# CCIG-Champalimaud/adell-mri

Hardware: AMD Instinct MI355X
Metric: volumes/sec 3D U-Net 128^3 2-ch seg (train step: fwd+loss+bwd+SGD) (higher is better)
Workload: dtype f32 (f16x3 split MFMA, fp32 accumulate); 1 GPU; BASELINE configs[1]: u-net-3d-resnet.yaml UNetPL, 2x128^3, batch 2/GPU, dice+focal, SGD-Nesterov; per_gpu_batch=2, parallelism=dp1, yaml=configs/u-net-3d-resnet.yaml, built_by=parse_config_unet -> get_segmentation_network('unet'), gradient_exchange=none (1 rank)

## Files before the change

adell_mri_amd/_lib.py:

```python
import ctypes
import os

_HERE = os.path.dirname(os.path.abspath(__file__))
LIB_PATH = os.environ.get("ADELL_HIP_LIBRARY") or os.path.join(_HERE, "libadellhip.so")

_lib = None

OK = 0
E_BADARG, E_UNSUPPORTED, E_HIP, E_NOMEM = -1, -2, -3, -4

ACT_IDS = {
    "identity": 0, "swish": 1, "silu": 1, "relu": 2, "leaky_relu": 3, "prelu": 4,
    "gelu": 5, "sigmoid": 6, "tanh": 7, "elu": 8,
}


class AdellHipError(RuntimeError):
    pass


class ConvDesc(ctypes.Structure):
    _fields_ = [(n, ctypes.c_int32) for n in (
        "N", "D", "H", "W", "C0", "C1", "Cout", "KD", "KH", "KW", "SD", "SH", "SW",
        "PD", "PH", "PW", "Do", "Ho", "Wo")]
# ... 93 lines not shown
    "adell_dice_focal_workspace": (_l, [_i, _l]),
    "adell_dice_focal_fwd": (_i, [_vp, _vp, _i, _l, _f, _f, _f, _f, _f, _vp, _vp, _vp, _vp, ctypes.c_size_t, _vp]),
    "adell_dice_focal_bwd": (_i, [_vp, _vp, _i, _l, _f, _f, _f, _f, _f, _vp, _f, _f, _vp, _vp]),
    "adell_dice_focal_bwd_dev": (_i, [_vp, _vp, _i, _l, _f, _f, _f, _f, _f, _vp, _vp, _vp, _vp, _vp]),
    "adell_class_sums_workspace": (_l, [_i, _l, _i]),
    "adell_class_sums_fwd": (_i, [_vp, _vp, _i, _l, _i, _vp, _vp, ctypes.c_size_t, _vp]),
    "adell_class_sums_bwd": (_i, [_vp, _vp, _i, _l, _i, _vp, _vp]),
    "adell_sgd_step": (_i, [_vp, _vp, _vp, _l, _f, _f, _f, _i, _i, _f, _vp]),
    "adell_adamw_step": (_i, [_vp, _vp, _vp, _vp, _l, _f, _f, _f, _f, _f, _l, _f, _vp]),
    "adell_adam_step": (_i, [_vp, _vp, _vp, _vp, _l, _f, _f, _f, _f, _f, _l, _f, _vp]),
    "adell_ema_update": (_i, [_vp, _vp, _l, _f, _vp]),
    "adell_layernorm_fwd": (_i, [_vp, _vp, _vp, _vp, _vp, _vp, _l, _i, _f, _vp]),
    "adell_layernorm_bwd_workspace": (_l, [_l, _i]),
    "adell_layernorm_bwd": (_i, [_vp] * 8 + [_l, _i, _vp, ctypes.c_size_t, _vp]),
    "adell_add_bcast": (_i, [_vp, _vp, _vp, _l, _l, _vp]),
    "adell_sum_bcast": (_i, [_vp, _vp, _l, _l, _vp]),
    "adell_attention_fwd": (_i, [_vp, _vp, _vp, _vp, _i, _i, _i, _i, _i, _f, _f, ctypes.c_ulonglong,
                                 ctypes.c_uint, _vp, _vp, _vp]),
    "adell_attention_bwd": (_i, [_vp, _vp, _vp, _vp, _i, _vp, _vp, _vp, _i, _i, _i, _i, _f, _f,
                                 ctypes.c_ulonglong, ctypes.c_uint, _vp, _vp, _vp, _vp]),
    "adell_attention_strided_ok": (_i, [_i, _i, _i]),
    "adell_attention_fwd_strided": (_i, [_vp, _vp, _vp, _vp, _i, _i, _i, _i, _i, _i, _vp, _f, _f,
                                         ctypes.c_ulonglong, ctypes.c_uint, _vp, _vp, _vp]),
    "adell_attention_bwd_strided": (_i, [_vp, _vp, _vp, _vp, _i, _vp, _vp, _vp, _i, _i, _i, _i, _i,
                                         _vp, _f, _f, ctypes.c_ulonglong, ctypes.c_uint, _vp, _vp,
                                         _vp, _vp]),
    "adell_copy_channels": (_i, [_vp, _vp, _l, _i, _i, _i, _i, _vp]),
    "adell_interp_nearest_fwd": (_i, [_vp, _vp] + [_i] * 8 + [_vp]),
    "adell_interp_nearest_bwd": (_i, [_vp, _vp] + [_i] * 8 + [_vp]),
    "adell_interp_linear_fwd": (_i, [_vp, _vp] + [_i] * 8 + [_f] * 3 + [_i, _vp]),
    "adell_interp_linear_bwd": (_i, [_vp, _vp] + [_i] * 8 + [_f] * 3 + [_i, _vp]),
    "adell_fold_x_taps": (_i, [_vp, _vp] + [_i] * 8 + [_vp]),
    "adell_scale_bc": (_i, [_vp, _vp, _vp, _i, _l, _i, _vp]),
    "adell_scale_bc_dscale_workspace_floats": (_l, [_i, _l, _i]),
    "adell_scale_bc_dscale": (_i, [_vp, _vp, _vp, _i, _l, _i, _vp, _vp]),
    "adell_cse_apply": (_i, [_vp, _vp, _vp, _vp, _vp, _vp, _i, _l, _i, _vp]),
    "adell_cse_apply_bwd_workspace_floats": (_l, [_i, _l, _i]),
    "adell_cse_apply_bwd": (_i, [_vp, _vp, _vp, _vp, _vp, _vp, _vp, _vp, _i, _l, _i, _vp, _vp]),
    "adell_bcast_nc": (_i, [_vp, _vp, _i, _l, _i, _f, _vp]),
    "adell_maxpool3d_fwd": (_i, [ctypes.POINTER(ConvDesc), _vp, _vp, _vp, _vp]),
    "adell_maxpool3d_bwd": (_i, [ctypes.POINTER(ConvDesc), _vp, _vp, _vp, _vp]),
    "adell_dwconv3d_fwd": (_i, [_i] * 8 + [_vp] * 5),
    "adell_dwconv3d_bwd_data": (_i, [_i] * 8 + [_vp] * 4),
    "adell_dwconv3d_bwd_weight_workspace_floats": (_l, [_i] * 8),
    "adell_dwconv3d_bwd_weight": (_i, [_i] * 8 + [_vp] * 6),
    "adell_vicreg_scratch_floats": (_l, [_i, _i]),
    "adell_vicreg_fwd": (_i, [_vp, _vp, _i, _i, _f, _f, _vp, _vp, _vp]),
    "adell_vicreg_bwd": (_i, [_vp, _vp, _i, _i, _f, _f, _vp, _vp, _vp, _vp, _vp]),
    "adell_convt_k2_applicable": (_i, [_i] * 6),
    "adell_convt_k2_fwd": (_i, [_i] * 6 + [_vp] * 5),
    "adell_convt_k2_bwd_data": (_i, [_i] * 6 + [_vp] * 4),
    "adell_convt_k2_wgrad_workspace": (_l, [_i] * 6),
    "adell_convt_k2_bwd_weight": (_i, [_i] * 6 + [_vp] * 5 + [ctypes.c_size_t, _vp]),
    "adell_convt_k221_applicable": (_i, [_i] * 6),
    "adell_convt_k221_fwd": (_i, [_i] * 6 + [_vp] * 5),
    "adell_convt_k221_bwd_data": (_i, [_i] * 6 + [_vp] * 4),
    "adell_convt_k221_wgrad_workspace": (_l, [_i] * 6),
    "adell_convt_k221_bwd_weight": (_i, [_i] * 6 + [_vp] * 5 + [ctypes.c_size_t, _vp]),
    "adell_conv_cinfold_applicable": (_i, [ctypes.POINTER(ConvDesc)]),
    "adell_conv_cinfold_ntiles": (_i, [ctypes.POINTER(ConvDesc)]),
    "adell_conv_cinfold_fwd": (_i, [ctypes.POINTER(ConvDesc)] + [_vp] * 5 + [_i, _vp]),
    "adell_conv_cinfold_fwd_f16x3": (_i, [ctypes.POINTER(ConvDesc)] + [_vp] * 5 + [_i, _vp]),
    "adell_conv_cinfold_wgrad_workspace": (_l, [ctypes.POINTER(ConvDesc)]),
    "adell_conv_cinfold_bwd_weight": (_i, [ctypes.POINTER(ConvDesc)] + [_vp] * 5
                                      + [ctypes.c_size_t, _vp]),
    "adell_conv_cinfold_bwd_weight_f16x3": (_i, [ctypes.POINTER(ConvDesc)] + [_vp] * 5
                                            + [ctypes.c_size_t, _vp]),
    "adell_conv_cinfold_dx_applicable": (_i, [ctypes.POINTER(ConvDesc)]),
    "adell_conv_cinfold_bwd_data": (_i, [ctypes.POINTER(ConvDesc)] + [_vp] * 4),
    "adell_conv_cinfold_bwd_data_f16x3": (_i, [ctypes.POINTER(ConvDesc)] + [_vp] * 4),
    "adell_pair_loss_scratch_floats": (_l, [_i, _i]),
    "adell_pair_loss_fwd": (_i, [_vp, _vp, _i, _i, _i, _f, _i, _vp, _vp, _vp]),
    "adell_pair_loss_bwd": (_i, [_vp, _vp, _i, _i, _i, _f, _i, _vp, _vp, _vp, _vp, _vp]),
    "adell_loco_loss_workspace": (_l, [_i, _l, _i]),
    "adell_loco_loss_fwd": (_i, [_vp, _vp, _i, _l, _i, _f, _f, _vp, _vp, ctypes.c_size_t, _vp]),
    "adell_loco_loss_bwd": (_i, [_vp, _vp, _vp, _i, _l, _i, _f, _f, _vp, _vp, _vp]),
    "adell_prelu_wgrad_workspace": (_l, [ctypes.POINTER(NormActDesc)]),
    "adell_prelu_wgrad": (_i, [ctypes.POINTER(NormActDesc)] + [_vp] * 8 + [ctypes.c_size_t, _vp]),
    "adell_convtranspose3d_fwd_f16x3": (_i, [_i] * 9 + [_vp] * 7),
    "adell_convtranspose3d_bwd_data_f16x3": (_i, [_i] * 9 + [_vp] * 6),
    "adell_convtranspose3d_f16x3_plan": (_i, [_i] * 9 + [_vp]),
    "adell_conv1_small_applicable": (_i, [ctypes.POINTER(ConvDesc)]),
    "adell_conv1_small_fwd": (_i, [ctypes.POINTER(ConvDesc)] + [_vp] * 6),
    "adell_conv1_small_bwd_data": (_i, [ctypes.POINTER(ConvDesc)] + [_vp] * 5),
    "adell_conv1_small_wgrad_workspace": (_l, [ctypes.POINTER(ConvDesc)]),
    "adell_conv1_small_bwd_weight": (_i, [ctypes.POINTER(ConvDesc)] + [_vp] * 6 + [ctypes.c_size_t, _vp]),
    "adell_conv_cin_small_applicable": (_i, [ctypes.POINTER(ConvDesc)]),
    "adell_conv_cin_small_ntiles": (_i, [ctypes.POINTER(ConvDesc)]),
    "adell_conv_cin_small_fwd": (_i, [ctypes.POINTER(ConvDesc)] + [_vp] * 5 + [_i, _vp]),
    "adell_conv_cin_small_bwd_data": (_i, [ctypes.POINTER(ConvDesc)] + [_vp] * 4),
    "adell_multi_copy": (_i, [_vp, _i, _vp, _vp]),
    "adell_grad_norm_workspace": (_l, [_i]),
    "adell_grad_norm_partials": (_i, [_vp, _l, _i, _vp, _i, _vp]),
    "adell_grad_norm_finalize": (_i, [_vp, _i, _i, _f, _f, _vp, _vp]),
    "adell_grad_scale_by": (_i, [_vp, _l, _vp, _vp]),
    "adell_multi_accumulate": (_i, [_vp, _i, _vp, _vp]),
    "adell_seg_confusion_workspace": (_l, [_l, _i]),
    "adell_seg_confusion_update": (_i, [_vp, _vp, _i, _l, _i, _l, _i, _vp, _l, _vp, _i, _vp]),
    "adell_seg_metric_compute": (_i, [_vp, _i, _i, _f, _vp, _vp]),
    "adell_cc_workspace": (_l, [_l, _i, _i, _i]),
    "adell_cc_label": (_i, [_vp, _l, _i, _i, _i, _i, _f, _vp, _vp, _vp, _l, _vp]),
    "adell_picai_tables_workspace": (_l, [_l, _i, _i, _i]),
    "adell_picai_tables_capacity": (_l, [_l, _i, _i, _i]),
    "adell_picai_tables": (_i, [_vp, _vp, _l, _i, _i, _i, _i, _f, _vp, _vp, _l, _vp, _l, _vp]),
    "adell_item_stats_workspace": (_l, [_i, _l]),
    "adell_item_stats": (_i, [_vp, _i, _l, _vp, _vp, ctypes.c_size_t, _vp]),
# ... 97 lines not shown
```

adell_mri_amd/csrc/convt_k2.hip:

```cpp
#include "common.h"

struct ConvTK2Args {
  const float* x;
  const float* w;
  const float* bias;
  const float* dy;
  float* y;
  float* dx;
  float* ws;
  float* wsdb;
  int N, D, H, W, Cin, Cout;
  int FX;
  long V;
  int ntiles;
};

__device__ __forceinline__ size_t adell_ctk2_fine(const ConvTK2Args& a, long v64, int fz, int fy) {
  const unsigned v = (unsigned)v64, W = (unsigned)a.W, H = (unsigned)a.H, D = (unsigned)a.D;
  const unsigned t1 = v / W, x = v - t1 * W;
  const unsigned t2 = t1 / H, y = t1 - t2 * H;
  const unsigned n = t2 / D, z = t2 - n * D;
  return (((size_t)n * 2 * D + 2 * z + fz) * 2 * H + 2 * y + fy) * (size_t)(a.FX * W) + (size_t)a.FX * x;
}

// ... 197 lines not shown
  float4 dbacc = make_float4(0.f, 0.f, 0.f, 0.f);
  auto fetch = [&](int t) {
    const long v0 = (long)t * 32;
    const int valid = (a.V - v0) < 32 ? (int)(a.V - v0) : 32;
    const size_t yrow = li < valid ? adell_ctk2_fine(a, v0 + li, fz, fy) * a.Cout : 0;
    adell_ctk2_fetch<32>(rx, valid, lane, a.x + (size_t)v0 * a.Cin + ci0, (size_t)li * a.Cin);
    adell_ctk2_fetch<32>(ry0, valid, lane, a.dy, yrow, co0);
    if constexpr (FX == 2) adell_ctk2_fetch<32>(ry1, valid, lane, a.dy, yrow, a.Cout + co0);
  };
  if ((int)blockIdx.x < a.ntiles) fetch(blockIdx.x);
  for (int t = blockIdx.x; t < a.ntiles; t += gridDim.x) {
    adell_ctk2_put<32>(tx, LDX, lane, rx);
    adell_ctk2_put<32>(tyl, LDY, lane, ry0);
    if constexpr (FX == 2) adell_ctk2_put<32>(tyl + 32, LDY, lane, ry1);
    if (do_db) {
#pragma unroll
      for (int u = 0; u < CtK2Regs<32>::PER; ++u) {
        dbacc.x += ry0.f[u].x; dbacc.y += ry0.f[u].y; dbacc.z += ry0.f[u].z; dbacc.w += ry0.f[u].w;
        if constexpr (FX == 2) {
          dbacc.x += ry1.f[u].x; dbacc.y += ry1.f[u].y; dbacc.z += ry1.f[u].z; dbacc.w += ry1.f[u].w;
        }
      }
    }
    __builtin_amdgcn_s_waitcnt(0xc07f);
    if (t + (int)gridDim.x < a.ntiles) fetch(t + gridDim.x);
#pragma unroll
    for (int s = 0; s < 16; ++s) {
      const int v = 2 * s + lh;
      const float av = tx[v * LDX + li];
#pragma unroll
      for (int fx = 0; fx < FX; ++fx)
        acc[fx] = __builtin_amdgcn_mfma_f32_32x32x2f32(av, tyl[v * LDY + fx * 32 + li], acc[fx],
                                                        0, 0, 0);
    }
  }
  float* out = a.ws + (((size_t)blockIdx.x * gridDim.y + blockIdx.y) * (4 * FX)) * 1024;
#pragma unroll
  for (int fx = 0; fx < FX; ++fx)
#pragma unroll
    for (int r = 0; r < 16; ++r) {
      const int row = (r & 3) + 8 * (r >> 2) + 4 * lh;
      out[(size_t)((fz * 2 + fy) * FX + fx) * 1024 + row * 32 + li] = acc[fx][r];
    }
  if (do_db) {
#pragma unroll
    for (int o = 8; o < 64; o <<= 1) {
      dbacc.x += __shfl_xor(dbacc.x, o, 64);
      dbacc.y += __shfl_xor(dbacc.y, o, 64);
      dbacc.z += __shfl_xor(dbacc.z, o, 64);
      dbacc.w += __shfl_xor(dbacc.w, o, 64);
    }
    if (lane < 8) {
      float* o = a.wsdb + ((size_t)blockIdx.x * 4 + wave) * a.Cout + co0 + 4 * lane;
      o[0] = dbacc.x; o[1] = dbacc.y; o[2] = dbacc.z; o[3] = dbacc.w;
    }
  }
}

__global__ __launch_bounds__(256) void adell_convt_k2_dw16_kernel(ConvTK2Args a) {
  constexpr int LDX = 33, LDY = 33;
  __shared__ float sx[4][32 * LDX];
  __shared__ float sy[4][32 * LDY];
  const int lane = threadIdx.x & 63, wave = threadIdx.x >> 6, li = lane & 31, lh = lane >> 5;
  const int fz = wave >> 1, fy = wave & 1;
  const int ci0 = blockIdx.y * 32;
  f32x16 acc;
#pragma unroll
  for (int r = 0; r < 16; ++r) acc[r] = 0.f;
  float* tx = sx[wave];
  float* tyl = sy[wave];
  CtK2Regs<32> rx, ry;
  const bool do_db = a.wsdb != nullptr && ci0 == 0;
  float4 dbacc = make_float4(0.f, 0.f, 0.f, 0.f);
  auto fetch = [&](int t) {
    const long v0 = (long)t * 32;
    const int valid = (a.V - v0) < 32 ? (int)(a.V - v0) : 32;
    const size_t yrow = li < valid ? adell_ctk2_fine(a, v0 + li, fz, fy) * 16 : 0;
    adell_ctk2_fetch<32>(rx, valid, lane, a.x + (size_t)v0 * a.Cin + ci0, (size_t)li * a.Cin);
    adell_ctk2_fetch<32>(ry, valid, lane, a.dy, yrow);
  };
  if ((int)blockIdx.x < a.ntiles) fetch(blockIdx.x);
  for (int t = blockIdx.x; t < a.ntiles; t += gridDim.x) {
    adell_ctk2_put<32>(tx, LDX, lane, rx);
    adell_ctk2_put<32>(tyl, LDY, lane, ry);
    if (do_db) {
#pragma unroll
      for (int u = 0; u < CtK2Regs<32>::PER; ++u) {
        dbacc.x += ry.f[u].x; dbacc.y += ry.f[u].y; dbacc.z += ry.f[u].z; dbacc.w += ry.f[u].w;
      }
    }
    __builtin_amdgcn_s_waitcnt(0xc07f);
    if (t + (int)gridDim.x < a.ntiles) fetch(t + gridDim.x);
#pragma unroll
    for (int s = 0; s < 16; ++s) {
      const int v = 2 * s + lh;
      acc = __builtin_amdgcn_mfma_f32_32x32x2f32(tx[v * LDX + li], tyl[v * LDY + li], acc, 0, 0, 0);
    }
  }
  float* out = a.ws + (((size_t)blockIdx.x * gridDim.y + blockIdx.y) * 4 + (fz * 2 + fy)) * 1024;
#pragma unroll
  for (int r = 0; r < 16; ++r) {
    const int row = (r & 3) + 8 * (r >> 2) + 4 * lh;
    out[row * 32 + li] = acc[r];
  }
  if (do_db) {
#pragma unroll
// ... 174 lines not shown
  return adell_convt_k2_wgrad_ws_impl(N, D, H, W, Cin, Cout, 1);
}

static int adell_convt_k2_bwd_weight_impl(int N, int D, int H, int W, int Cin, int Cout, int FX,
                                          const float* x, const float* dy, float* dw, float* db,
                                          void* workspace, size_t workspace_bytes, void* stream) {
  ADELL_REQUIRE(x && dy && dw && workspace && adell_convt_k2_ok(N, D, H, W, Cin, Cout, FX),
                "convt_k2_bwd_weight: factor-2 transposed conv with 32 / 64 channels expected");
  ADELL_REQUIRE((((uintptr_t)x | (uintptr_t)dy) & 15) == 0,
                "convt_k2_bwd_weight: x and dy must be 16-byte aligned");
  ADELL_REQUIRE((long)workspace_bytes >= adell_convt_k2_wgrad_ws_impl(N, D, H, W, Cin, Cout, FX),
                "convt_k2_bwd_weight: workspace too small");
  ConvTK2Args a = {};
  adell_ctk2_fill(&a, N, D, H, W, Cin, Cout, FX);
  a.x = x; a.dy = dy; a.ws = (float*)workspace;
  const int blocks = adell_ctk2_blocks(a, 2);
  hipStream_t st = (hipStream_t)stream;
  if (Cout == 16) {
    a.wsdb = db ? a.ws + (size_t)blocks * (Cin / 32) * 4 * 1024 : nullptr;
    hipLaunchKernelGGL(adell_convt_k2_dw16_kernel, dim3((unsigned)blocks, (unsigned)(Cin / 32)), dim3(256),
                       0, st, a);
    const long outs16 = (long)Cin * 16 * 8 + (db ? 16 : 0);
    hipLaunchKernelGGL(adell_convt_k2_dw16_reduce_kernel, dim3((unsigned)((outs16 + 3) / 4)), dim3(256),
                       0, st, (const float*)workspace, blocks, Cin, dw, (const float*)a.wsdb, db);
    ADELL_CHECK_HIP(hipGetLastError());
    return ADELL_OK;
  }
  const int F = 4 * FX;
  a.wsdb = db ? a.ws + (size_t)blocks * (Cin / 32) * (Cout / 32) * F * 1024 : nullptr;
  dim3 grid((unsigned)blocks, (unsigned)((Cin / 32) * (Cout / 32)));
  if (FX == 2)
    hipLaunchKernelGGL(adell_convt_k2_dw_kernel<2>, grid, dim3(256), 0, st, a);
  else
    hipLaunchKernelGGL(adell_convt_k2_dw_kernel<1>, grid, dim3(256), 0, st, a);
  const long outs = (long)Cin * Cout * F + (db ? Cout : 0);
  hipLaunchKernelGGL(adell_convt_k2_dw_reduce_kernel, dim3((unsigned)((outs + 3) / 4)), dim3(256), 0,
                     st, (const float*)workspace, blocks, Cin, Cout, dw, (const float*)a.wsdb, db, F);
  ADELL_CHECK_HIP(hipGetLastError());
  return ADELL_OK;
}

extern "C" int adell_convt_k2_bwd_weight(int N, int D, int H, int W, int Cin, int Cout,
                                         const float* x, const float* dy, float* dw, float* db,
                                         void* workspace, size_t workspace_bytes, void* stream) {
  return adell_convt_k2_bwd_weight_impl(N, D, H, W, Cin, Cout, 2, x, dy, dw, db, workspace,
                                        workspace_bytes, stream);
}
extern "C" int adell_convt_k221_bwd_weight(int N, int D, int H, int W, int Cin, int Cout,
                                           const float* x, const float* dy, float* dw, float* db,
                                           void* workspace, size_t workspace_bytes, void* stream) {
  return adell_convt_k2_bwd_weight_impl(N, D, H, W, Cin, Cout, 1, x, dy, dw, db, workspace,
                                        workspace_bytes, stream);
}
```

adell_mri_amd/functional.py:

```python
import itertools
import os
import weakref

import numpy as np
import torch
import torch.distributed as dist

from . import _lib, ops

_dropout_counter = itertools.count(1)

CONV_PRECISION = os.environ.get("ADELL_CONV_PRECISION", "f16x3")
FLAGS = {"s2class_always": bool(os.environ.get("ADELL_S2CLASS_ALWAYS")),
         "no_s2class": bool(os.environ.get("ADELL_NO_S2CLASS")),
         "no_fold": bool(os.environ.get("ADELL_NO_FOLD")),
         "no_adn_fuse": bool(os.environ.get("ADELL_NO_ADN_FUSE")),
         "no_lowrank": bool(os.environ.get("ADELL_NO_LOWRANK")),
         "wgrad_stream": os.environ.get("ADELL_WGRAD_STREAM", "1") != "0",
         "no_rows": bool(os.environ.get("ADELL_NO_ROWS")),
         "no_pointwise_gemm": bool(os.environ.get("ADELL_NO_POINTWISE_GEMM")),
         "no_seq_attention": bool(os.environ.get("ADELL_NO_SEQ_ATTENTION")),
         "no_mlp_fuse": not bool(os.environ.get("ADELL_MLP_FUSE")),
         "mlp_min_elems": int(os.environ.get("ADELL_MLP_MIN_ELEMS", str(1 << 20))),
         "no_cinfold_wgrad_f16": bool(os.environ.get("ADELL_NO_CINFOLD_WGRAD_F16"))}


def set_conv_precision(mode):
    global CONV_PRECISION
    if mode not in ("f16x3", "fp32"):
        raise ValueError("conv precision must be 'f16x3' or 'fp32'")
    CONV_PRECISION = mode
    _sync_dw_precision()


def _sync_dw_precision():
    from . import _lib
    if os.path.exists(_lib.LIB_PATH) and not os.environ.get("ADELL_DW_NOMFMA"):
        _lib.lib().adell_set_tuning(b"dw_nomfma", 1 if CONV_PRECISION == "fp32" else 0)


if CONV_PRECISION == "fp32":
    _sync_dw_precision()


class _Ref:

    __slots__ = ("obj",)

    def __init__(self, obj):
        self.obj = obj


_PACK_REG = {}
_PACK_BATCH = {"epoch": -1, "sig": None, "table": None, "blocks": 0}


class _PackFence:

    __slots__ = ("stream", "event")

    def __init__(self):
        self.stream = ops._stream().value
        self.event = torch.cuda.Event()
        self.event.record()

    def order(self):
        if ops._stream().value != self.stream:
            torch.cuda.current_stream().wait_event(self.event)


def _pack_tag(w):
    return (w._version, w.data_ptr(), ops.WEIGHT_EPOCH)


def _repack_registered():
    live = []
    for key, ent in list(_PACK_REG.items()):
# ... 626 lines not shown
    adn = _adn_sites_of(x0, x1, weight, stride, padding)
    rows0 = getattr(x0, "_adell_rows", None)
    rows1 = getattr(x1, "_adell_rows", None) if x1 is not None else None
    conf = (stride, padding, want_stats, _Ref(weight), carry_in, carry_out, carry_x0, carry_cat,
            adn, rows0, rows1)
    Cin = x0.shape[1] + (0 if x1 is None else x1.shape[1])
    small1 = ops.conv1_small_ok(weight, Cin, stride, padding, residual)
    if small1:
        wp = None
        site = getattr(x0, "_adell_site", None) if getattr(x0, "_adell_single", False) else None
        if (site is not None and x1 is None and carry_in is None and carry_x0 is None
                and not grad_observed(x0)
                and not FLAGS["no_adn_fuse"] and not FLAGS["no_lowrank"]
                and torch.is_grad_enabled() and ops.norm_act_lowrank_ok(x0, weight.shape[0])):
            conf = conf[:8] + (("lowrank", site),) + conf[9:]
    elif ops.conv_cin_small_ok(weight, x0, x1, stride, padding, residual):
        wp = "cin_small"
    elif ops.conv_cinfold_ok(weight, x0, x1, stride, padding, residual):
        wp = "cinfold"
    elif (CONV_PRECISION == "f16x3" and x1 is None and weight.dim() == 5 and x0.shape[1] <= 4
          and 3 <= weight.shape[4] and weight.shape[4] * x0.shape[1] <= 16
          and stride == (1, 1, 1) and not FLAGS["no_fold"]):
        wp = ("fold", _packed_folded(weight))
    else:
        wp = _packed(weight, 0)
    y, part = _Conv3dFn.apply(x0, x1, weight, bias, residual, wp, conf)
    if want_stats and part.numel() > 0:
        y._adell_partials = part
    return y


class _ConvT3dFn(torch.autograd.Function):
    @staticmethod
    def forward(ctx, x, weight, bias, wp, wref):
        factors = tuple(weight.shape[2:])
        ctx.k2 = wp is None
        if ctx.k2:
            y = ops.convt_k2_fwd(x, weight, bias)
        else:
            y = ops.convtranspose3d_fwd(x, wp, bias, weight.shape[1], factors)
        ctx.save_for_backward(x, weight)
        ctx.has_bias = bias is not None
        ctx.bias_ref = _Ref(bias)
        ctx.wref = wref
        ctx.factors = factors
        return y

    @staticmethod
    def backward(ctx, dy):
        x, weight = ctx.saved_tensors
        need = ctx.needs_input_grad
        dy = ops.ndhwc(dy)
        dx = dw = db = None
        if need[0]:
            dx = (ops.convt_k2_bwd_data(dy, weight) if ctx.k2 else
                  ops.convtranspose3d_bwd_data(dy, _packed(ctx.wref.obj, 3), weight.shape[0],
                                               ctx.factors))
        want_db = ctx.has_bias and need[2]

        def weight_grads():
            dw = db = None
            if need[1] and ctx.k2 and want_db:
                dw, db = ops.convt_k2_bwd_weight(x, dy, want_db=True, factors=ctx.factors)
            elif need[1]:
                dw = (ops.convt_k2_bwd_weight(x, dy, factors=ctx.factors) if ctx.k2 else
                      ops.convtranspose3d_bwd_weight(x, dy, ctx.factors))
            if want_db and db is None:
                db = ops.bias_grad(dy)
            return dw, db

        if (need[1] or want_db) and _side_ok(ctx.wref.obj, ctx.bias_ref.obj):
            dw, db = side_run(weight_grads, (x, dy))
        else:
            dw, db = weight_grads()
        return dx, dw, db, None, None


def conv_transpose3d(x, weight, bias=None):
    wp = None if (x.dim() == 5 and ops.convt_k2_ok(x.shape, weight)) else _packed(weight, 2)
    _note_use(weight)
    return _ConvT3dFn.apply(x, weight, bias, wp, _Ref(weight))


conv_transpose3d_k2s2 = conv_transpose3d


class _NormDropActFn(torch.autograd.Function):
    @staticmethod
    def forward(ctx, x, mean, rstd, gamma, beta, act_w, conf):
        act, act_p, per_item, drop_p, seed, offset, site, split_exp, _group = conf
        if site is not None:
            out, mask = ops.norm_act_fwd(x, mean, rstd, act, gamma=gamma, beta=beta, act_w=act_w,
                                         act_p=act_p, stats_per_item=per_item, drop_p=drop_p,
                                         seed=seed, rng_offset=offset, want_mask=True,
                                         split_exp=split_exp)
            site.x, site.mean, site.rstd, site.mask = x, mean, rstd, mask
        else:
            out = ops.norm_act_fwd(x, mean, rstd, act, gamma=gamma, beta=beta, act_w=act_w,
                                   act_p=act_p, stats_per_item=per_item, drop_p=drop_p, seed=seed,
                                   rng_offset=offset, split_exp=split_exp)
        ctx.save_for_backward(x, mean, rstd, gamma, beta, act_w)
        ctx.conf = conf
        return out

    @staticmethod
    def backward(ctx, dout):
        x, mean, rstd, gamma, beta, act_w = ctx.saved_tensors
        act, act_p, per_item, drop_p, seed, offset, site, _split_exp, group = ctx.conf
        if site is not None:
            fused, part, poff = site.fused, site.part, site.poff
            site.fused, site.part = False, None
# ... 948 lines not shown
```

adell_mri_amd/ops.py:

```python
import collections
import ctypes
import math
import os

import torch

from . import _lib
from ._lib import ACT_IDS, AdellHipError, ConvDesc, NormActDesc, check


class KernelTimer:

    def __init__(self, only=None):
        self.records = []
        self._agg = None
        self.only = None if only is None else set(only)
        self.active = True

    def start(self):
        e = torch.cuda.Event(enable_timing=True)
        e.record()
        return e

    def stop(self, name, flops, e0, tag=None, nbytes=0.0, kernels=1):
# ... 751 lines not shown
    N, Cin, D, H, W = x.shape
    Cout = weight.shape[1]
    f = tuple(weight.shape[2:])
    y = new_act(N, Cout, f[0] * D, f[1] * H, f[2] * W, x.device)
    wc = weight.contiguous()
    fn = _convt_k2_fns(f)[1]
    nf = f[0] * f[1] * f[2]
    check(_timed("adell_convt_k2_kernel", 2.0 * nf * N * D * H * W * Cin * Cout,
                 lambda: fn(N, D, H, W, Cin, Cout, _ptr(x), _ptr(wc), _ptr(bias), _ptr(y), _stream()),
                 f"convT fwd {Cin}->{Cout} in {D}x{H}x{W} f{f[0]}{f[1]}{f[2]}",
                 4.0 * (x.numel() + y.numel())))
    return y


def convt_k2_bwd_data(dy, weight):
    _require_cuda(dy, weight)
    dy = ndhwc(dy)
    N, Cout, D2, H2, W2 = dy.shape
    Cin = weight.shape[0]
    f = tuple(weight.shape[2:])
    D, H, W = D2 // f[0], H2 // f[1], W2 // f[2]
    dx = new_act(N, Cin, D, H, W, dy.device)
    wc = weight.contiguous()
    fn = _convt_k2_fns(f)[2]
    nf = f[0] * f[1] * f[2]
    check(_timed("adell_convt_k2_kernel", 2.0 * nf * N * D * H * W * Cin * Cout,
                 lambda: fn(N, D, H, W, Cin, Cout, _ptr(dy), _ptr(wc), _ptr(dx), _stream()),
                 f"convT dgrad {Cin}->{Cout} in {D}x{H}x{W} f{f[0]}{f[1]}{f[2]}",
                 4.0 * (dy.numel() + dx.numel())))
    return dx


def convt_k2_bwd_weight(x, dy, want_db=False, factors=(2, 2, 2)):
    _require_cuda(x, dy)
    x, dy = ndhwc(x), ndhwc(dy)
    N, Cin, D, H, W = x.shape
    Cout = dy.shape[1]
    f = tuple(factors)
    fns = _convt_k2_fns(f)
    nbytes = fns[3](N, D, H, W, Cin, Cout)
    check(min(nbytes, 0))
    ws = _workspace(nbytes, x.device)
    dw = torch.empty((Cin, Cout, *f), device=x.device, dtype=torch.float32)
    db = torch.empty(Cout, device=x.device, dtype=torch.float32) if want_db else None
    nf = f[0] * f[1] * f[2]
    check(_timed("adell_convt_k2_kernel", 2.0 * nf * N * D * H * W * Cin * Cout,
                 lambda: fns[4](N, D, H, W, Cin, Cout, _ptr(x), _ptr(dy), _ptr(dw), _ptr(db), _ptr(ws),
                                ws.numel() * 4, _stream()),
                 f"convT wgrad {Cin}->{Cout} in {D}x{H}x{W} f{f[0]}{f[1]}{f[2]}",
                 4.0 * (x.numel() + dy.numel())))
    return (dw, db) if want_db else dw


def convtranspose3d_k2s2_bwd_weight(x, dy):
    return convtranspose3d_bwd_weight(x, dy, (2, 2, 2))


def convtranspose3d_fwd(x, w_packed, bias, Cout, factors=(2, 2, 2)):
    _require_cuda(x, bias)
    x = ndhwc(x)
    N, Cin, D, H, W = x.shape
    fd, fh, fw = factors
    y = new_act(N, Cout, fd * D, fh * H, fw * W, x.device)
    flops = 2.0 * N * D * H * W * Cin * Cout * fd * fh * fw
    if isinstance(w_packed, SplitWeight):
        check(_timed("adell_conv_igemm_f16_kernel", flops,
                     lambda: _lib.lib().adell_convtranspose3d_fwd_f16x3(
                         N, D, H, W, Cin, Cout, fd, fh, fw, _ptr(x), _ptr(w_packed.halfs),
                         _ptr(w_packed.scale), _ptr(bias), _ptr(y), None, _stream()),
                     f"convT fwd {Cin}->{Cout} in {D}x{H}x{W} f{fd}{fh}{fw}",
                     4.0 * (x.numel() + y.numel())))
        return y
    _require_cuda(w_packed)
    check(_timed("adell_conv_igemm_kernel", flops, lambda: _lib.lib().adell_convtranspose3d_fwd(
        N, D, H, W, Cin, Cout, fd, fh, fw, _ptr(x), _ptr(w_packed), _ptr(bias), _ptr(y),
        _stream())))
    return y


def convtranspose3d_bwd_data(dy, w_packed_bwd, Cin, factors=(2, 2, 2)):
    _require_cuda(dy)
    dy = ndhwc(dy)
    N, Cout, D2, H2, W2 = dy.shape
    fd, fh, fw = factors
    D, H, W = D2 // fd, H2 // fh, W2 // fw
    dx = new_act(N, Cin, D, H, W, dy.device)
    flops = 2.0 * N * D * H * W * Cin * Cout * fd * fh * fw
    if isinstance(w_packed_bwd, SplitWeight):
        check(_timed("adell_conv_igemm_f16_kernel", flops,
                     lambda: _lib.lib().adell_convtranspose3d_bwd_data_f16x3(
                         N, D, H, W, Cin, Cout, fd, fh, fw, _ptr(dy), _ptr(w_packed_bwd.halfs),
                         _ptr(w_packed_bwd.scale), _ptr(dx), None, _stream()),
                     f"convT dgrad {Cin}->{Cout} in {D}x{H}x{W} f{fd}{fh}{fw}",
                     4.0 * (dy.numel() + dx.numel())))
        return dx
    _require_cuda(w_packed_bwd)
    check(_timed("adell_conv_igemm_kernel", flops, lambda: _lib.lib().adell_convtranspose3d_bwd_data(
        N, D, H, W, Cin, Cout, fd, fh, fw, _ptr(dy), _ptr(w_packed_bwd), _ptr(dx), _stream())))
    return dx


def convtranspose3d_k2s2_fwd(x, w_packed, bias, Cout):
    return convtranspose3d_fwd(x, w_packed, bias, Cout, (2, 2, 2))


def convtranspose3d_k2s2_bwd_data(dy, w_packed_bwd, Cin):
# ... 1257 lines not shown
```

include/adell_hip.h:

```cpp
#ifndef ADELL_HIP_H
#define ADELL_HIP_H

#include <stddef.h>
#include <stdint.h>

#ifdef __cplusplus
extern "C" {
#endif
#if defined(__GNUC__) || defined(__clang__)
#pragma GCC visibility push(default)
#endif

#define ADELL_OK 0
#define ADELL_E_BADARG (-1)
#define ADELL_E_UNSUPPORTED (-2)
#define ADELL_E_HIP (-3)
#define ADELL_E_NOMEM (-4)

#define ADELL_ABI_VERSION 2

enum {
  ADELL_ACT_IDENTITY = 0,
  ADELL_ACT_SILU = 1,
  ADELL_ACT_RELU = 2,
// ... 326 lines not shown
                    const float* acc, float* y, int N, long V, int C, void* stream);
long adell_cse_apply_bwd_workspace_floats(int N, long V, int C);
int adell_cse_apply_bwd(const float* x, const float* dy, const float* s, const float* c,
                        const float* inv, float* dx, float* ds, float* dc, int N, long V, int C,
                        float* workspace, void* stream);
int adell_bcast_nc(const float* g, float* out, int N, long V, int C, float scale, void* stream);

int adell_maxpool3d_fwd(const adell_conv3d_desc* d, const float* x, float* y,
                        int32_t* argmax, void* stream);
int adell_maxpool3d_bwd(const adell_conv3d_desc* d, const float* dy, const int32_t* argmax,
                        float* dx, void* stream);

int adell_dwconv3d_fwd(int N, int C, int D, int H, int W, int KD, int KH, int KW,
                       const float* x, const float* w, const float* bias, float* y,
                       void* stream);
int adell_dwconv3d_bwd_data(int N, int C, int D, int H, int W, int KD, int KH, int KW,
                            const float* dy, const float* w, float* dx, void* stream);
long adell_dwconv3d_bwd_weight_workspace_floats(int N, int C, int D, int H, int W, int KD, int KH,
                                                int KW);
int adell_dwconv3d_bwd_weight(int N, int C, int D, int H, int W, int KD, int KH, int KW,
                              const float* x, const float* dy, float* dw, float* db,
                              float* workspace, void* stream);
long adell_vicreg_scratch_floats(int B, int D);
int adell_vicreg_fwd(const float* x1, const float* x2, int B, int D, float min_var, float eps,
                     float* scratch, float* out3, void* stream);
int adell_vicreg_bwd(const float* x1, const float* x2, int B, int D, float min_var, float eps,
                     const float* scratch, const float* g3, float* dx1, float* dx2,
                     void* stream);

long adell_pair_loss_scratch_floats(int B, int D);
int adell_pair_loss_fwd(const float* x1, const float* x2, int B, int D, int kind,
                        float temperature, int apply_relu, float* scratch, float* loss,
                        void* stream);
int adell_pair_loss_bwd(const float* x1, const float* x2, int B, int D, int kind,
                        float temperature, int apply_relu, const float* scratch, const float* g,
                        float* dx1, float* dx2, void* stream);

long adell_loco_loss_workspace(int B, long S, int C);
int adell_loco_loss_fwd(const float* f1, const float* f2, int B, long S, int C, float temperature,
                        float eps, float* loss, void* workspace, size_t workspace_bytes,
                        void* stream);
int adell_loco_loss_bwd(const float* f1, const float* f2, const float* gloss, int B, long S, int C,
                        float temperature, float eps, float* df1, float* df2, void* stream);

int adell_convt_k2_applicable(int N, int D, int H, int W, int Cin, int Cout);
int adell_convt_k2_fwd(int N, int D, int H, int W, int Cin, int Cout, const float* x,
                       const float* w, const float* bias, float* y, void* stream);
int adell_convt_k2_bwd_data(int N, int D, int H, int W, int Cin, int Cout, const float* dy,
                            const float* w, float* dx, void* stream);
long adell_convt_k2_wgrad_workspace(int N, int D, int H, int W, int Cin, int Cout);
int adell_convt_k2_bwd_weight(int N, int D, int H, int W, int Cin, int Cout, const float* x,
                              const float* dy, float* dw, float* db, void* workspace,
                              size_t workspace_bytes, void* stream);
int adell_convt_k221_applicable(int N, int D, int H, int W, int Cin, int Cout);
int adell_convt_k221_fwd(int N, int D, int H, int W, int Cin, int Cout, const float* x,
                         const float* w, const float* bias, float* y, void* stream);
int adell_convt_k221_bwd_data(int N, int D, int H, int W, int Cin, int Cout, const float* dy,
                              const float* w, float* dx, void* stream);
long adell_convt_k221_wgrad_workspace(int N, int D, int H, int W, int Cin, int Cout);
int adell_convt_k221_bwd_weight(int N, int D, int H, int W, int Cin, int Cout, const float* x,
                                const float* dy, float* dw, float* db, void* workspace,
                                size_t workspace_bytes, void* stream);

int adell_conv_cinfold_applicable(const adell_conv3d_desc* d);
int adell_conv_cinfold_ntiles(const adell_conv3d_desc* d);
int adell_conv_cinfold_fwd(const adell_conv3d_desc* d, const float* x, const float* w,
                           const float* bias, float* y, float* stat_partials, int partial_rows,
                           void* stream);
int adell_conv_cinfold_fwd_f16x3(const adell_conv3d_desc* d, const float* x, const float* w,
                                 const float* bias, float* y, float* stat_partials, int partial_rows,
                           void* stream);
long adell_conv_cinfold_wgrad_workspace(const adell_conv3d_desc* d);
int adell_conv_cinfold_bwd_weight(const adell_conv3d_desc* d, const float* x, const float* dy,
                                  float* dw, float* db, void* workspace, size_t workspace_bytes,
                                  void* stream);
int adell_conv_cinfold_bwd_weight_f16x3(const adell_conv3d_desc* d, const float* x, const float* dy,
                                        float* dw, float* db, void* workspace,
                                        size_t workspace_bytes, void* stream);
int adell_conv_cinfold_dx_applicable(const adell_conv3d_desc* d);
int adell_conv_cinfold_bwd_data(const adell_conv3d_desc* d, const float* dy, const float* w,
                                float* dx, void* stream);
int adell_conv_cinfold_bwd_data_f16x3(const adell_conv3d_desc* d, const float* dy, const float* w,
                                      float* dx, void* stream);

int adell_conv1_small_applicable(const adell_conv3d_desc* d);
int adell_conv1_small_fwd(const adell_conv3d_desc* d, const float* x0, const float* x1,
                          const float* w, const float* bias, float* y, void* stream);
int adell_conv1_small_bwd_data(const adell_conv3d_desc* d, const float* dy, const float* w,
                               float* dx0, float* dx1, void* stream);
long adell_conv1_small_wgrad_workspace(const adell_conv3d_desc* d);
int adell_conv1_small_bwd_weight(const adell_conv3d_desc* d, const float* x0, const float* x1,
                                 const float* dy, float* dw, float* db, void* workspace,
                                 size_t workspace_bytes, void* stream);

int adell_conv_cin_small_applicable(const adell_conv3d_desc* d);
int adell_conv_cin_small_ntiles(const adell_conv3d_desc* d);
int adell_conv_cin_small_fwd(const adell_conv3d_desc* d, const float* x, const float* w,
                             const float* bias, float* y, float* stat_partials, int partial_rows,
                           void* stream);
int adell_conv_cin_small_bwd_data(const adell_conv3d_desc* d, const float* dy, const float* w,
                                  float* dx, void* stream);

int adell_multi_copy(const long* table, int rows, float* dst, void* stream);

long adell_grad_norm_workspace(int runs);
int adell_grad_norm_partials(const float* g, long n, int norm_inf, double* partials, int run,
// ... 132 lines not shown
```

Baseline: 61.72 volumes/s.

## Fuse transposed-conv k2 data and weight gradients into one kernel pass

Adds a fused backward kernel for factor-2 transposed convolutions with 32 output channels. It reads each dy and x tile once and computes both dx, via cross-wave reduction through shared memory, and the per-block weight-gradient partials. A separate fold kernel reduces those partials to dw and db, optionally on a side stream. This removes the second full read of dy that separate dgrad and wgrad kernels needed, at the cost of extra shared-memory synchronisation and higher register pressure. Experimental variants can be picked with environment variables.

```diff
diff --git a/adell_mri_amd/_lib.py b/adell_mri_amd/_lib.py
--- a/adell_mri_amd/_lib.py
+++ b/adell_mri_amd/_lib.py
@@ -169,6 +169,9 @@
     "adell_convt_k2_bwd_data": (_i, [_i] * 6 + [_vp] * 4),
     "adell_convt_k2_wgrad_workspace": (_l, [_i] * 6),
     "adell_convt_k2_bwd_weight": (_i, [_i] * 6 + [_vp] * 5 + [ctypes.c_size_t, _vp]),
+    "adell_convt_k2_bwd_fused_applicable": (_i, [_i] * 6),
+    "adell_convt_k2_bwd_fused": (_i, [_i] * 6 + [_vp] * 4 + [_i, _vp, ctypes.c_size_t, _vp]),
+    "adell_convt_k2_wgrad_fold": (_i, [_i] * 6 + [_vp, ctypes.c_size_t, _vp, _vp, _vp]),
     "adell_convt_k221_applicable": (_i, [_i] * 6),
     "adell_convt_k221_fwd": (_i, [_i] * 6 + [_vp] * 5),
     "adell_convt_k221_bwd_data": (_i, [_i] * 6 + [_vp] * 4),
diff --git a/adell_mri_amd/csrc/convt_k2.hip b/adell_mri_amd/csrc/convt_k2.hip
--- a/adell_mri_amd/csrc/convt_k2.hip
+++ b/adell_mri_amd/csrc/convt_k2.hip
@@ -273,6 +273,229 @@
     }
     if (lane < 8) {
       float* o = a.wsdb + ((size_t)blockIdx.x * 4 + wave) * a.Cout + co0 + 4 * lane;
+      o[0] = dbacc.x; o[1] = dbacc.y; o[2] = dbacc.z; o[3] = dbacc.w;
+    }
+  }
+}
+
+__global__ __launch_bounds__(256) __attribute__((amdgpu_waves_per_eu(2, 2))) void adell_convt_k2_dxdw_kernel(ConvTK2Args a) {
+  constexpr int COUT = 32, KW = 2 * COUT, LDY = KW + 1, LDX = 33, KS = KW / 2;
+  __shared__ float sy[4][32 * LDY];
+  __shared__ float sx[4][32 * LDX];
+  __shared__ float sred[3 * 32 * 33];
+  const int lane = threadIdx.x & 63, wave = threadIdx.x >> 6, li = lane & 31, lh = lane >> 5;
+  const int fz = wave >> 1, fy = wave & 1, ci0 = blockIdx.y * 32, ci = ci0 + li;
+  float bw[KS];
+#pragma unroll
+  for (int s = 0; s < KS; ++s) {
+    const int k = 2 * s + lh, fx = k / COUT, co = k - fx * COUT;
+    bw[s] = a.w[((size_t)ci * COUT + co) * 8 + (fz * 2 + fy) * 2 + fx];
+  }
+  f32x16 accw[2];
+#pragma unroll
+  for (int fx = 0; fx < 2; ++fx)
+#pragma unroll
+    for (int r = 0; r < 16; ++r) accw[fx][r] = 0.f;
+  float* ty = sy[wave];
+  float* tx = sx[wave];
+  CtK2Regs<32> rx, ry0, ry1;
+  const bool do_db = a.wsdb != nullptr && ci0 == 0;
+  float4 dbacc = make_float4(0.f, 0.f, 0.f, 0.f);
+  auto fetch = [&](int t) {
+    const long v0 = (long)t * 32;
+    const int valid = (a.V - v0) < 32 ? (int)(a.V - v0) : 32;
+    const size_t yrow = li < valid ? adell_ctk2_fine(a, v0 + li, fz, fy) * COUT : 0;
+    adell_ctk2_fetch<32>(rx, valid, lane, a.x + (size_t)v0 * a.Cin + ci0, (size_t)li * a.Cin);
+    adell_ctk2_fetch<32>(ry0, valid, lane, a.dy, yrow, 0);
+    adell_ctk2_fetch<32>(ry1, valid, lane, a.dy, yrow, COUT);
+  };
+  if ((int)blockIdx.x < a.ntiles) fetch(blockIdx.x);
+  for (int t = blockIdx.x; t < a.ntiles; t += gridDim.x) {
+    const long v0 = (long)t * 32;
+    const int valid = (a.V - v0) < 32 ? (int)(a.V - v0) : 32;
+    adell_ctk2_put<32>(tx, LDX, lane, rx);
+    adell_ctk2_put<32>(ty, LDY, lane, ry0);
+    adell_ctk2_put<32>(ty + 32, LDY, lane, ry1);
+    if (do_db) {
+#pragma unroll
+      for (int u = 0; u < CtK2Regs<32>::PER; ++u) {
+        dbacc.x += ry0.f[u].x; dbacc.y += ry0.f[u].y; dbacc.z += ry0.f[u].z; dbacc.w += ry0.f[u].w;
+        dbacc.x += ry1.f[u].x; dbacc.y += ry1.f[u].y; dbacc.z += ry1.f[u].z; dbacc.w += ry1.f[u].w;
+      }
+    }
+    __builtin_amdgcn_s_waitcnt(0xc07f);
+    if (t + (int)gridDim.x < a.ntiles) fetch(t + gridDim.x);
+    f32x16 accd;
+#pragma unroll
+    for (int r = 0; r < 16; ++r) accd[r] = 0.f;
+#pragma unroll
+    for (int s = 0; s < KS; ++s)
+      accd = __builtin_amdgcn_mfma_f32_32x32x2f32(ty[li * LDY + 2 * s + lh], bw[s], accd, 0, 0, 0);
+#pragma unroll
+    for (int s = 0; s < 16; ++s) {
+      const int v = 2 * s + lh;
+      const float av = tx[v * LDX + li];
+#pragma unroll
+      for (int fx = 0; fx < 2; ++fx)
+        accw[fx] = __builtin_amdgcn_mfma_f32_32x32x2f32(av, ty[v * LDY + fx * 32 + li], accw[fx],
+                                                         0, 0, 0);
+    }
+    if (wave > 0) {
+#pragma unroll
+      for (int r = 0; r < 16; ++r)
+        sred[((wave - 1) * 32 + (r & 3) + 8 * (r >> 2) + 4 * lh) * 33 + li] = accd[r];
+    }
+    __syncthreads();
+    if (wave == 0) {
+#pragma unroll
+      for (int r = 0; r < 16; ++r) {
+        const int row = (r & 3) + 8 * (r >> 2) + 4 * lh;
+        if (row < valid)
+          a.dx[(size_t)(v0 + row) * a.Cin + ci] =
+              ((accd[r] + sred[row * 33 + li]) + sred[(32 + row) * 33 + li]) +
+              sred[(64 + row) * 33 + li];
+      }
+    }
+    __syncthreads();
+  }
+  float* out = a.ws + (((size_t)blockIdx.x * gridDim.y + blockIdx.y) * 8) * 1024;
+#pragma unroll
+  for (int fx = 0; fx < 2; ++fx)
+#pragma unroll
+    for (int r = 0; r < 16; ++r) {
+      const int row = (r & 3) + 8 * (r >> 2) + 4 * lh;
+      out[(size_t)((fz * 2 + fy) * 2 + fx) * 1024 + row * 32 + li] = accw[fx][r];
+    }
+  if (do_db) {
+#pragma unroll
+    for (int o = 8; o < 64; o <<= 1) {
+      dbacc.x += __shfl_xor(dbacc.x, o, 64);
+      dbacc.y += __shfl_xor(dbacc.y, o, 64);
+      dbacc.z += __shfl_xor(dbacc.z, o, 64);
+      dbacc.w += __shfl_xor(dbacc.w, o, 64);
+    }
+    if (lane < 8) {
+      float* o = a.wsdb + ((size_t)blockIdx.x * 4 + wave) * COUT + 4 * lane;
+      o[0] = dbacc.x; o[1] = dbacc.y; o[2] = dbacc.z; o[3] = dbacc.w;
+    }
+  }
+}
+
+template <bool IL>
+__global__ __launch_bounds__(256) __attribute__((amdgpu_waves_per_eu(2, 2))) void adell_convt_k2_dxdw2_kernel(ConvTK2Args a) {
+  constexpr int COUT = 32, KW = 2 * COUT, LDY = KW + 1, LDX = 33, KS = KW / 2;
+  __shared__ float sy[4][32 * LDY];
+  __shared__ float sx[4][32 * LDX];
+  const int lane = threadIdx.x & 63, wave = threadIdx.x >> 6, li = lane & 31, lh = lane >> 5;
+  const int fz = wave >> 1, fy = wave & 1, ci0 = blockIdx.y * 32, ci = ci0 + li;
+  float bw[KS];
+#pragma unroll
+  for (int s = 0; s < KS; ++s) {
+    const int k = 2 * s + lh, fx = k / COUT, co = k - fx * COUT;
+    bw[s] = a.w[((size_t)ci * COUT + co) * 8 + (fz * 2 + fy) * 2 + fx];
+  }
+  f32x16 accw[2];
+#pragma unroll
+  for (int fx = 0; fx < 2; ++fx)
+#pragma unroll
+    for (int r = 0; r < 16; ++r) accw[fx][r] = 0.f;
+  float* ty = sy[wave];
+  float* tx = sx[wave];
+  CtK2Regs<32> rx, ry0, ry1;
+  const bool do_db = a.wsdb != nullptr && ci0 == 0;
+  float4 dbacc = make_float4(0.f, 0.f, 0.f, 0.f);
+  auto fetch = [&](int t) {
+    const long v0 = (long)t * 32;
+    const int valid = (a.V - v0) < 32 ? (int)(a.V - v0) : 32;
+    const size_t yrow = li < valid ? adell_ctk2_fine(a, v0 + li, fz, fy) * COUT : 0;
+    adell_ctk2_fetch<32>(rx, valid, lane, a.x + (size_t)v0 * a.Cin + ci0, (size_t)li * a.Cin);
+    adell_ctk2_fetch<32>(ry0, valid, lane, a.dy, yrow, 0);
+    adell_ctk2_fetch<32>(ry1, valid, lane, a.dy, yrow, COUT);
+  };
+  auto fold = [&](int t) {
+    const long v0 = (long)t * 32;
+    const int valid = (a.V - v0) < 32 ? (int)(a.V - v0) : 32;
+#pragma unroll
+    for (int j = 0; j < 4; ++j) {
+      int row = 8 * wave + 4 * lh + j;
+      row = row < valid ? row : valid - 1;
+      const float v = ((sx[0][row * LDX + li] + sx[1][row * LDX + li]) + sx[2][row * LDX + li]) +
+                      sx[3][row * LDX + li];
+      a.dx[(size_t)(v0 + row) * a.Cin + ci] = v;
+    }
+  };
+  auto tile = [&](int t) {
+    adell_ctk2_put<32>(tx, LDX, lane, rx);
+    adell_ctk2_put<32>(ty, LDY, lane, ry0);
+    adell_ctk2_put<32>(ty + 32, LDY, lane, ry1);
+    if (do_db) {
+#pragma unroll
+      for (int u = 0; u < CtK2Regs<32>::PER; ++u) {
+        dbacc.x += ry0.f[u].x; dbacc.y += ry0.f[u].y; dbacc.z += ry0.f[u].z; dbacc.w += ry0.f[u].w;
+        dbacc.x += ry1.f[u].x; dbacc.y += ry1.f[u].y; dbacc.z += ry1.f[u].z; dbacc.w += ry1.f[u].w;
+      }
+    }
+    __builtin_amdgcn_s_waitcnt(0xc07f);
+    fetch(t + (int)gridDim.x < a.ntiles ? t + (int)gridDim.x : t);
+    f32x16 accd;
+#pragma unroll
+    for (int r = 0; r < 16; ++r) accd[r] = 0.f;
+    if constexpr (IL) {
+#pragma unroll
+      for (int s = 0; s < 16; ++s) {
+        const int v = 2 * s + lh;
+        const float av = tx[v * LDX + li];
+        accd = __builtin_amdgcn_mfma_f32_32x32x2f32(ty[li * LDY + 4 * s + lh], bw[2 * s], accd, 0, 0, 0);
+        accw[0] = __builtin_amdgcn_mfma_f32_32x32x2f32(av, ty[v * LDY + li], accw[0], 0, 0, 0);
+        accd = __builtin_amdgcn_mfma_f32_32x32x2f32(ty[li * LDY + 4 * s + 2 + lh], bw[2 * s + 1], accd,
+                                                    0, 0, 0);
+        accw[1] = __builtin_amdgcn_mfma_f32_32x32x2f32(av, ty[v * LDY + 32 + li], accw[1], 0, 0, 0);
+      }
+    } else {
+#pragma unroll
+      for (int s = 0; s < KS; ++s)
+        accd = __builtin_amdgcn_mfma_f32_32x32x2f32(ty[li * LDY + 2 * s + lh], bw[s], accd, 0, 0, 0);
+#pragma unroll
+      for (int s = 0; s < 16; ++s) {
+        const int v = 2 * s + lh;
+        const float av = tx[v * LDX + li];
+#pragma unroll
+        for (int fx = 0; fx < 2; ++fx)
+          accw[fx] = __builtin_amdgcn_mfma_f32_32x32x2f32(av, ty[v * LDY + fx * 32 + li], accw[fx],
+                                                           0, 0, 0);
+      }
+    }
+#pragma unroll
+    for (int r = 0; r < 16; ++r) tx[((r & 3) + 8 * (r >> 2) + 4 * lh) * LDX + li] = accd[r];
+    __syncthreads();
+  };
+  int t = blockIdx.x;
+  fetch(t);
+  tile(t);
+  for (t += gridDim.x; t < a.ntiles; t += gridDim.x) {
+    fold(t - (int)gridDim.x);
+    __syncthreads();
+    tile(t);
+  }
+  fold(t - (int)gridDim.x);
+  float* out = a.ws + (((size_t)blockIdx.x * gridDim.y + blockIdx.y) * 8) * 1024;
+#pragma unroll
+  for (int fx = 0; fx < 2; ++fx)
+#pragma unroll
+    for (int r = 0; r < 16; ++r) {
+      const int row = (r & 3) + 8 * (r >> 2) + 4 * lh;
+      out[(size_t)((fz * 2 + fy) * 2 + fx) * 1024 + row * 32 + li] = accw[fx][r];
+    }
+  if (do_db) {
+#pragma unroll
+    for (int o = 8; o < 64; o <<= 1) {
+      dbacc.x += __shfl_xor(dbacc.x, o, 64);
+      dbacc.y += __shfl_xor(dbacc.y, o, 64);
+      dbacc.z += __shfl_xor(dbacc.z, o, 64);
+      dbacc.w += __shfl_xor(dbacc.w, o, 64);
+    }
+    if (lane < 8) {
+      float* o = a.wsdb + ((size_t)blockIdx.x * 4 + wave) * COUT + 4 * lane;
       o[0] = dbacc.x; o[1] = dbacc.y; o[2] = dbacc.z; o[3] = dbacc.w;
     }
   }
@@ -553,3 +776,55 @@
   return adell_convt_k2_bwd_weight_impl(N, D, H, W, Cin, Cout, 1, x, dy, dw, db, workspace,
                                         workspace_bytes, stream);
 }
+
+extern "C" int adell_convt_k2_bwd_fused_applicable(int N, int D, int H, int W, int Cin, int Cout) {
+  return adell_convt_k2_ok(N, D, H, W, Cin, Cout) && Cout == 32 ? 1 : 0;
+}
+
+extern "C" int adell_convt_k2_bwd_fused(int N, int D, int H, int W, int Cin, int Cout,
+                                        const float* x, const float* dy, const float* w, float* dx,
+                                        int want_db, void* workspace, size_t workspace_bytes,
+                                        void* stream) {
+  ADELL_REQUIRE(x && dy && w && dx && workspace &&
+                    adell_convt_k2_bwd_fused_applicable(N, D, H, W, Cin, Cout),
+                "convt_k2_bwd_fused: factor-2 transposed conv with 32 / 64 -> 32 channels expected");
+  ADELL_REQUIRE((((uintptr_t)x | (uintptr_t)dy) & 15) == 0,
+                "convt_k2_bwd_fused: x and dy must be 16-byte aligned");
+  ADELL_REQUIRE((long)workspace_bytes >= adell_convt_k2_wgrad_ws_impl(N, D, H, W, Cin, Cout, 2),
+                "convt_k2_bwd_fused: workspace too small");
+  ConvTK2Args a = {};
+  adell_ctk2_fill(&a, N, D, H, W, Cin, Cout, 2);
+  a.x = x; a.dy = dy; a.w = w; a.dx = dx; a.ws = (float*)workspace;
+  const int blocks = adell_ctk2_blocks(a, 2);
+  a.wsdb = want_db ? a.ws + (size_t)blocks * (Cin / 32) * 8 * 1024 : nullptr;
+  if (getenv("ADELL_EXP_DXDW_V0"))
+    hipLaunchKernelGGL(adell_convt_k2_dxdw_kernel, dim3((unsigned)blocks, (unsigned)(Cin / 32)),
+                       dim3(256), 0, (hipStream_t)stream, a);
+  else if (getenv("ADELL_EXP_DXDW_IL"))
+    hipLaunchKernelGGL(adell_convt_k2_dxdw2_kernel<true>, dim3((unsigned)blocks, (unsigned)(Cin / 32)),
+                       dim3(256), 0, (hipStream_t)stream, a);
+  else
+    hipLaunchKernelGGL(adell_convt_k2_dxdw2_kernel<false>, dim3((unsigned)blocks, (unsigned)(Cin / 32)),
+                       dim3(256), 0, (hipStream_t)stream, a);
+  ADELL_CHECK_HIP(hipGetLastError());
+  return ADELL_OK;
+}
+
+extern "C" int adell_convt_k2_wgrad_fold(int N, int D, int H, int W, int Cin, int Cout,
+                                         const void* workspace, size_t workspace_bytes, float* dw,
+                                         float* db, void* stream) {
+  ADELL_REQUIRE(workspace && dw && adell_convt_k2_bwd_fused_applicable(N, D, H, W, Cin, Cout),
+                "convt_k2_wgrad_fold: factor-2 transposed conv with 32 / 64 -> 32 channels expected");
+  ADELL_REQUIRE((long)workspace_bytes >= adell_convt_k2_wgrad_ws_impl(N, D, H, W, Cin, Cout, 2),
+                "convt_k2_wgrad_fold: workspace too small");
+  ConvTK2Args a = {};
+  adell_ctk2_fill(&a, N, D, H, W, Cin, Cout, 2);
+  const int blocks = adell_ctk2_blocks(a, 2);
+  const float* ws = (const float*)workspace;
+  const float* wsdb = db ? ws + (size_t)blocks * (Cin / 32) * 8 * 1024 : nullptr;
+  const long outs = (long)Cin * Cout * 8 + (db ? Cout : 0);
+  hipLaunchKernelGGL(adell_convt_k2_dw_reduce_kernel, dim3((unsigned)((outs + 3) / 4)), dim3(256), 0,
+                     (hipStream_t)stream, ws, blocks, Cin, Cout, dw, wsdb, db, 8);
+  ADELL_CHECK_HIP(hipGetLastError());
+  return ADELL_OK;
+}
diff --git a/adell_mri_amd/functional.py b/adell_mri_amd/functional.py
--- a/adell_mri_amd/functional.py
+++ b/adell_mri_amd/functional.py
@@ -22,7 +22,8 @@
          "no_seq_attention": bool(os.environ.get("ADELL_NO_SEQ_ATTENTION")),
          "no_mlp_fuse": not bool(os.environ.get("ADELL_MLP_FUSE")),
          "mlp_min_elems": int(os.environ.get("ADELL_MLP_MIN_ELEMS", str(1 << 20))),
-         "no_cinfold_wgrad_f16": bool(os.environ.get("ADELL_NO_CINFOLD_WGRAD_F16"))}
+         "no_cinfold_wgrad_f16": bool(os.environ.get("ADELL_NO_CINFOLD_WGRAD_F16")),
+         "no_convt_bwd_fuse": bool(os.environ.get("ADELL_NO_CONVT_BWD_FUSE"))}
 
 
 def set_conv_precision(mode):
@@ -755,11 +756,24 @@
         need = ctx.needs_input_grad
         dy = ops.ndhwc(dy)
         dx = dw = db = None
+        want_db = ctx.has_bias and need[2]
+        if (ctx.k2 and need[0] and need[1] and not FLAGS["no_convt_bwd_fuse"]
+                and ops.convt_k2_bwd_fused_ok(x.shape, weight)):
+            dx, part = ops.convt_k2_bwd_fused(x, dy, weight, want_db)
+
+            def fold():
+                out = ops.convt_k2_wgrad_fold(part, tuple(x.shape), weight.shape[1], want_db)
+                return out if want_db else (out, None)
+
+            if _side_ok(ctx.wref.obj, ctx.bias_ref.obj):
+                dw, db = side_run(fold, (part,))
+            else:
+                dw, db = fold()
+            return dx, dw, db, None, None
         if need[0]:
             dx = (ops.convt_k2_bwd_data(dy, weight) if ctx.k2 else
                   ops.convtranspose3d_bwd_data(dy, _packed(ctx.wref.obj, 3), weight.shape[0],
                                                ctx.factors))
-        want_db = ctx.has_bias and need[2]
 
         def weight_grads():
             dw = db = None
diff --git a/adell_mri_amd/ops.py b/adell_mri_amd/ops.py
--- a/adell_mri_amd/ops.py
+++ b/adell_mri_amd/ops.py
@@ -827,6 +827,46 @@
     return (dw, db) if want_db else dw
 
 
+def convt_k2_bwd_fused_ok(x_shape, weight):
+    if not convt_k2_ok(x_shape, weight) or tuple(weight.shape[2:]) != (2, 2, 2):
+        return False
+    N, _, D, H, W = x_shape
+    return bool(_lib.lib().adell_convt_k2_bwd_fused_applicable(N, D, H, W, weight.shape[0],
+                                                               weight.shape[1]))
+
+
+def convt_k2_bwd_fused(x, dy, weight, want_db=False):
+    _require_cuda(x, dy, weight)
+    x, dy = ndhwc(x), ndhwc(dy)
+    N, Cin, D, H, W = x.shape
+    Cout = dy.shape[1]
+    L = _lib.lib()
+    nbytes = L.adell_convt_k2_wgrad_workspace(N, D, H, W, Cin, Cout)
+    check(min(nbytes, 0))
+    ws = _workspace(nbytes, x.device)
+    dx = new_act(N, Cin, D, H, W, dy.device)
+    wc = weight.contiguous()
+    check(_timed("adell_convt_k2_kernel", 2 * 2.0 * 8 * N * D * H * W * Cin * Cout,
+                 lambda: L.adell_convt_k2_bwd_fused(N, D, H, W, Cin, Cout, _ptr(x), _ptr(dy), _ptr(wc),
+                                                    _ptr(dx), int(bool(want_db)), _ptr(ws),
+                                                    ws.numel() * 4, _stream()),
+                 f"convT dgrad+wgrad {Cin}->{Cout} in {D}x{H}x{W} f222",
+                 4.0 * (dy.numel() + x.numel() + dx.numel())))
+    return dx, ws
+
+
+def convt_k2_wgrad_fold(ws, x_shape, Cout, want_db=False):
+    N, Cin, D, H, W = x_shape
+    dw = torch.empty((Cin, Cout, 2, 2, 2), device=ws.device, dtype=torch.float32)
+    db = torch.empty(Cout, device=ws.device, dtype=torch.float32) if want_db else None
+    check(_timed("adell_convt_k2_kernel", 0.0,
+                 lambda: _lib.lib().adell_convt_k2_wgrad_fold(N, D, H, W, Cin, Cout, _ptr(ws),
+                                                              ws.numel() * 4, _ptr(dw), _ptr(db),
+                                                              _stream()),
+                 f"convT wgrad fold {Cin}->{Cout} in {D}x{H}x{W} f222", 4.0 * ws.numel()))
+    return (dw, db) if want_db else dw
+
+
 def convtranspose3d_k2s2_bwd_weight(x, dy):
     return convtranspose3d_bwd_weight(x, dy, (2, 2, 2))
 
diff --git a/include/adell_hip.h b/include/adell_hip.h
--- a/include/adell_hip.h
+++ b/include/adell_hip.h
@@ -402,6 +402,12 @@
 int adell_convt_k2_bwd_weight(int N, int D, int H, int W, int Cin, int Cout, const float* x,
                               const float* dy, float* dw, float* db, void* workspace,
                               size_t workspace_bytes, void* stream);
+int adell_convt_k2_bwd_fused_applicable(int N, int D, int H, int W, int Cin, int Cout);
+int adell_convt_k2_bwd_fused(int N, int D, int H, int W, int Cin, int Cout, const float* x,
+                             const float* dy, const float* w, float* dx, int want_db,
+                             void* workspace, size_t workspace_bytes, void* stream);
+int adell_convt_k2_wgrad_fold(int N, int D, int H, int W, int Cin, int Cout, const void* workspace,
+                              size_t workspace_bytes, float* dw, float* db, void* stream);
 int adell_convt_k221_applicable(int N, int D, int H, int W, int Cin, int Cout);
 int adell_convt_k221_fwd(int N, int D, int H, int W, int Cin, int Cout, const float* x,
                          const float* w, const float* bias, float* y, void* stream);
```

Result: no change. 61.80 volumes/s (median of 6 runs) (+0.1%).
